# SimonsRoad/gf-pl-slam

Hardware: AMD Instinct MI355X
Metric: stereo frames/sec (2k ORB + 500 LBD, 10 GN iters) (higher is better)
Workload: dtype f64

## Files before the change

gf-pl-slam_amd/csrc/gfpl_abi.hip:

```cpp
#include <hip/hip_runtime.h>

#include <algorithm>
#include <atomic>
#include <cmath>
#include <mutex>
#include <cstdio>
#include <cstdlib>
#include <cstring>
#include <vector>

#include "../../include/gfpl.h"
#include "gfpl_kernels.hpp"

using namespace gfpl;

#define GFPL_NEV 10

struct gfpl_ctx {
    int device = 0;
    hipStream_t stream = nullptr;
    bool own_stream = false;
    gfpl_camera cam{};
    gfpl_config cfg{};
    bool has_cam = false, has_cfg = false;
    bool timing = false;
    hipEvent_t ev[GFPL_NEV]{};
    float stage_ms[7]{};
    std::vector<gfpl_seqbatch*> sbs;
    std::atomic<int> n_detectors{0};
    std::mutex host_mu;
};

struct gfpl_seqbatch {
    gfpl_ctx* ctx = nullptr;
    int B = 0, kp_cap = 0, kl_cap = 0, mpt_cap = 0, mls_cap = 0;
    void* base = nullptr;
    int64_t bytes = 0;
    DevFrame slot[2];
    int prev_slot = 0;
    bool initialized = false;
    bool has_curr = false;
    DevTrack tr{};
    DevScratch scr{};
    void* stage[2] = {nullptr, nullptr};
    size_t stage_bytes[2] = {0, 0};
    gfpl_frames stage_view[2]{};
    hipStream_t copy = nullptr;
    hipEvent_t ev_ready[2]{}, ev_free[2]{};
    bool ready_pending[2] = {false, false}, free_recorded[2] = {false, false};
    hipEvent_t ev_ticket[16]{};
    int64_t n_tickets = 0;
    int32_t* last_n_pt = nullptr;
    int32_t* last_n_ls = nullptr;
    PyrBuild* pyrb = nullptr;
    int last_cut_mode = -1;
};

struct gfpl_event {
    int device = 0;
    hipEvent_t ev = nullptr;
    int64_t records = 0;
};

int gfpl_ctx_device(const gfpl_ctx* c) { return c->device; }
void* gfpl_ctx_stream(const gfpl_ctx* c) { return (void*)c->stream; }
const gfpl_camera* gfpl_ctx_camera(const gfpl_ctx* c) { return c->has_cam ? &c->cam : nullptr; }
int64_t gfpl_event_records(const gfpl_event* e) { return e->records; }
void gfpl_ctx_attach(gfpl_ctx* c) { c->n_detectors.fetch_add(1); }
void gfpl_ctx_detach(gfpl_ctx* c) { c->n_detectors.fetch_sub(1); }


namespace {

#define HIPCHK(x)                                                  \
    do {                                                            \
        hipError_t e_ = (x);                                        \
        if (e_ != hipSuccess) {                                     \
            std::fprintf(stderr, "gfpl: %s failed: %s\n", #x, hipGetErrorString(e_)); \
            return GFPL_E_HIP;                                      \
        }                                                           \
    } while (0)

int debug_fill_byte() {
    const char* e = getenv("GFPL_DEBUG_FILL");
    return e ? (int)(strtol(e, nullptr, 0) & 0xFF) : 0;
}

template <typename F, typename H, typename V>
void frame_fields(F& f, H& o, V& v) {
    v.pt(f.pt.pl, o.pt_pl, 2); v.pt(f.pt.pl_obs, o.pt_pl_obs, 2);
    v.pt(f.pt.disp, o.pt_disp, 1); v.pt(f.pt.P, o.pt_P, 3); v.pt(f.pt.sigma2, o.pt_sigma2, 1);
    v.pt(f.pt.idx, o.pt_idx, 1); v.pt(f.pt.level, o.pt_level, 1); v.pt(f.pt.inlier, o.pt_inlier, 1);
    v.pt(f.pt.desc, o.pdesc, 32); v.count(f.pt.n);
    v.ls(f.ls.spl, o.ls_spl, 2); v.ls(f.ls.epl, o.ls_epl, 2);
    v.ls(f.ls.spl_obs, o.ls_spl_obs, 2); v.ls(f.ls.epl_obs, o.ls_epl_obs, 2);
    v.ls(f.ls.sdisp, o.ls_sdisp, 1); v.ls(f.ls.edisp, o.ls_edisp, 1);
    v.ls(f.ls.sdisp_obs, o.ls_sdisp_obs, 1); v.ls(f.ls.edisp_obs, o.ls_edisp_obs, 1);
    v.ls(f.ls.angle, o.ls_angle, 1); v.ls(f.ls.sigma2, o.ls_sigma2, 1);
    v.ls(f.ls.sP, o.ls_sP, 3); v.ls(f.ls.eP, o.ls_eP, 3);
    v.ls(f.ls.le, o.ls_le, 3); v.ls(f.ls.le_obs, o.ls_le_obs, 3);
    v.ls(f.ls.covS, o.ls_covS, 9); v.ls(f.ls.covE, o.ls_covE, 9);
    v.ls(f.ls.cut, o.ls_cut, 2); v.ls(f.ls.invcov, o.ls_invcov, 36);
    v.ls(f.ls.idx, o.ls_idx, 1); v.ls(f.ls.level, o.ls_level, 1); v.ls(f.ls.inlier, o.ls_inlier, 1);
    v.ls(f.ls.desc, o.ldesc, 32); v.count(f.ls.n);
    v.seq(f.pose.Tfw, o.Tfw, 16); v.seq(f.pose.DT, o.DT, 16);
    v.seq(f.pose.DT_cov, o.DT_cov, 36); v.seq(f.pose.Tfw_cov, o.Tfw_cov, 36);
    v.seq(f.pose.DT_cov_eig, o.DT_cov_eig, 6);
    v.seq(f.pose.err_norm, &o.err_norm, 1); v.seq(f.pose.time_stamp, &o.time_stamp, 1);
}

struct SlotCarve {
    Carver& c;
    size_t B, P, L;
    template <typename T, typename U> void pt(T*& d, U, int w) { d = c.take<T>(P * w); }
// ... 240 lines not shown

int gfpl_event_record(gfpl_event* e, gfpl_ctx* c) {
    if (!e || !c || e->device != c->device) return GFPL_E_INVALID;
    HIPCHK(hipEventRecord(e->ev, c->stream));
    ++e->records;
    return GFPL_OK;
}

int gfpl_event_wait(gfpl_ctx* c, gfpl_event* e) {
    if (!e || !c || e->device != c->device) return GFPL_E_INVALID;
    HIPCHK(hipStreamWaitEvent(c->stream, e->ev, 0));
    return GFPL_OK;
}

int gfpl_event_synchronize(gfpl_event* e) {
    if (!e) return GFPL_E_INVALID;
    HIPCHK(hipEventSynchronize(e->ev));
    return GFPL_OK;
}

int gfpl_set_camera(gfpl_ctx* c, const gfpl_camera* cam) {
    if (!c || !cam || cam->n_levels < 1 || cam->n_levels > GFPL_MAX_LEVELS) return GFPL_E_INVALID;
    if (!c->sbs.empty() || c->n_detectors.load() != 0) return GFPL_E_STATE;
    int64_t need = 0;
    for (int i = 0; i < cam->n_levels; ++i) {
        if (cam->lvl_cols[i] < 1 || cam->lvl_rows[i] < 1 || cam->lvl_offset[i] < 0) return GFPL_E_INVALID;
        if (cam->lvl_cols[i] > GFPL_MAX_IMAGE_DIM || cam->lvl_rows[i] > GFPL_MAX_IMAGE_DIM) return GFPL_E_INVALID;
        need = std::max<int64_t>(need, cam->lvl_offset[i] + (int64_t)cam->lvl_cols[i] * cam->lvl_rows[i]);
    }
    if (cam->pyr_bytes < need + GFPL_PYR_TAIL) return GFPL_E_INVALID;
    if (cam->pyr_bytes % 4 != 0) return GFPL_E_INVALID;
    c->cam = *cam;
    c->has_cam = true;
    return GFPL_OK;
}

int gfpl_set_config(gfpl_ctx* c, const gfpl_config* cfg) {
    if (!c || !cfg) return GFPL_E_INVALID;
    int e = cfg_supported(*cfg);
    if (e) return e;
    for (const gfpl_seqbatch* sb : c->sbs)
        if (cfg->max_point_match_num > sb->mpt_cap || cfg->max_line_match_num > sb->mls_cap) return GFPL_E_CAPACITY;
    c->cfg = *cfg;
    c->has_cfg = true;
    return GFPL_OK;
}

int gfpl_get_camera(const gfpl_ctx* c, gfpl_camera* cam) {
    if (!c || !cam || !c->has_cam) return GFPL_E_INVALID;
    *cam = c->cam;
    return GFPL_OK;
}

int gfpl_get_config(const gfpl_ctx* c, gfpl_config* cfg) {
    if (!c || !cfg) return GFPL_E_INVALID;
    *cfg = c->cfg;
    return GFPL_OK;
}

int gfpl_synchronize(gfpl_ctx* c) {
    if (!c) return GFPL_E_INVALID;
    HIPCHK(hipStreamSynchronize(c->stream));
    return GFPL_OK;
}

int gfpl_seqbatch_create(gfpl_ctx* c, int batch, int kp_cap, int kl_cap, gfpl_seqbatch** out) {
    if (!c || !out || batch < 1 || kp_cap < 2 || kl_cap < 2 || kp_cap > 8192 || kl_cap > 2048 || !c->has_cam)
        return GFPL_E_INVALID;
    HIPCHK(hipSetDevice(c->device));
    gfpl_seqbatch* sb = new gfpl_seqbatch();
    sb->ctx = c;
    sb->B = batch;
    sb->kp_cap = (kp_cap + 1) & ~1;
    sb->kl_cap = (kl_cap + 1) & ~1;
    sb->mpt_cap = c->cfg.max_point_match_num;
    sb->mls_cap = c->cfg.max_line_match_num;
    Carver dry;
// ... 13 lines not shown
}

int gfpl_seqbatch_destroy(gfpl_seqbatch* sb) {
    if (!sb) return GFPL_E_INVALID;
    (void)hipStreamSynchronize(sb->ctx->stream);
    auto& v = sb->ctx->sbs;
    v.erase(std::remove(v.begin(), v.end(), sb), v.end());
    if (sb->copy) (void)hipStreamSynchronize(sb->copy);
    if (sb->base) (void)hipFree(sb->base);
    for (int k = 0; k < 2; ++k) {
        if (sb->stage[k]) (void)hipFree(sb->stage[k]);
        if (sb->ev_ready[k]) (void)hipEventDestroy(sb->ev_ready[k]);
        if (sb->ev_free[k]) (void)hipEventDestroy(sb->ev_free[k]);
    }
    for (hipEvent_t e : sb->ev_ticket)
        if (e) (void)hipEventDestroy(e);
    if (sb->copy) (void)hipStreamDestroy(sb->copy);
    pyrbuild_destroy(sb->pyrb);
    delete sb;
    return GFPL_OK;
}

int64_t gfpl_seqbatch_bytes(const gfpl_seqbatch* sb) { return sb ? sb->bytes : 0; }

int gfpl_initialize(gfpl_seqbatch* sb, const gfpl_frames* in) {
    if (!sb) return GFPL_E_INVALID;
    int e = check_in(sb, in);
    if (e) return e;
    const int slot = in_acquire(sb, in);
    if (slot == -2) return GFPL_E_HIP;
    KParams p = params(sb, in);
    p.curr = sb->slot[sb->prev_slot];
    HIPCHK(launch_init(p, sb->ctx->stream));
    sb->initialized = true;
    sb->has_curr = false;
    return in_release(sb, in, slot);
}

int gfpl_stereo_points(gfpl_seqbatch* sb, const gfpl_frames* in) {
    if (!sb) return GFPL_E_INVALID;
    if (!sb->initialized) return GFPL_E_STATE;
    int e = check_in(sb, in);
    if (e) return e;
    const int slot = in_acquire(sb, in);
    if (slot == -2) return GFPL_E_HIP;
    HIPCHK(launch_stereo_points(params(sb, in), sb->ctx->stream));
    sb->has_curr = true;
    return in_release(sb, in, slot);
}

int gfpl_stereo_lines(gfpl_seqbatch* sb, const gfpl_frames* in) {
    if (!sb) return GFPL_E_INVALID;
    if (!sb->initialized) return GFPL_E_STATE;
    int e = check_in(sb, in);
    if (e) return e;
    const int slot = in_acquire(sb, in);
    if (slot == -2) return GFPL_E_HIP;
    HIPCHK(launch_stereo_lines(params(sb, in), sb->ctx->stream));
    sb->has_curr = true;
    return in_release(sb, in, slot);
}

int gfpl_line_uncertainty(gfpl_seqbatch* sb) {
    if (!sb) return GFPL_E_INVALID;
    if (!sb->initialized) return GFPL_E_STATE;
    HIPCHK(launch_line_uncertainty(params(sb, nullptr), sb->ctx->stream));
    return GFPL_OK;
}

int gfpl_cross_points(gfpl_seqbatch* sb) {
    if (!sb) return GFPL_E_INVALID;
    if (!sb->initialized || !sb->has_curr) return GFPL_E_STATE;
    HIPCHK(launch_cross_points(params(sb, nullptr), sb->ctx->stream));
    return GFPL_OK;
}

int gfpl_cross_lines(gfpl_seqbatch* sb) {
    if (!sb) return GFPL_E_INVALID;
    if (!sb->initialized || !sb->has_curr) return GFPL_E_STATE;
    HIPCHK(launch_cross_lines(params(sb, nullptr), sb->ctx->stream));
    return GFPL_OK;
}

int gfpl_line_cut(gfpl_seqbatch* sb) {
    if (!sb) return GFPL_E_INVALID;
    if (!sb->initialized || !sb->has_curr) return GFPL_E_STATE;
    sb->last_cut_mode = sb->ctx->cfg.cut_proof;
    HIPCHK(launch_line_cut(params(sb, nullptr), sb->ctx->stream, nullptr));
    return GFPL_OK;
}

int gfpl_insert_stereo_pair(gfpl_seqbatch* sb, const gfpl_frames* in) {
    if (!sb) return GFPL_E_INVALID;
    if (!sb->initialized) return GFPL_E_STATE;
    int e = check_in(sb, in);
    if (e) return e;
    gfpl_ctx* c = sb->ctx;
    const int slot = in_acquire(sb, in);
    if (slot == -2) return GFPL_E_HIP;
    KParams p = params(sb, in);
    tmark(c, 0);
    HIPCHK(launch_stereo_points(p, c->stream));
    tmark(c, 1);
    HIPCHK(launch_stereo_lines(p, c->stream));
    tmark(c, 2);
    if (c->cfg.use_line_conf_cut) HIPCHK(launch_line_uncertainty(p, c->stream));
    HIPCHK(launch_cross_points(p, c->stream));
    tmark(c, 3);
    HIPCHK(launch_cross_lines(p, c->stream));
    tmark(c, 4);
    sb->last_cut_mode = c->cfg.use_line_conf_cut ? c->cfg.cut_proof : -1;
    if (c->cfg.use_line_conf_cut)
        HIPCHK(launch_line_cut(p, c->stream, c->timing ? &c->ev[7] : nullptr));
    HIPCHK(launch_step_bytes(p, c->stream));
    tmark(c, 5);
    sb->has_curr = true;
    return in_release(sb, in, slot);
}

int gfpl_optimize_pose(gfpl_seqbatch* sb) {
    if (!sb) return GFPL_E_INVALID;
    if (!sb->initialized || !sb->has_curr) return GFPL_E_STATE;
    HIPCHK(launch_pose(params(sb, nullptr), sb->ctx->stream, sb->ctx->timing ? sb->ctx->ev[9] : nullptr));
    tmark(sb->ctx, 6);
    return GFPL_OK;
}

int gfpl_need_new_kf(gfpl_seqbatch* sb, int32_t* flags) {
    if (!sb) return GFPL_E_INVALID;
    if (!sb->initialized || !sb->has_curr) return GFPL_E_STATE;
    HIPCHK(launch_need_kf(params(sb, nullptr), sb->ctx->stream));
    if (flags) {
        HIPCHK(hipMemcpyAsync(flags, sb->tr.kf_flag, sizeof(int32_t) * (size_t)sb->B, hipMemcpyDeviceToHost,
                              sb->ctx->stream));
        HIPCHK(hipStreamSynchronize(sb->ctx->stream));
    }
    return GFPL_OK;
}

int gfpl_curr_frame_is_kf(gfpl_seqbatch* sb, const int32_t* mask) {
    if (!sb) return GFPL_E_INVALID;
    if (!sb->initialized || !sb->has_curr) return GFPL_E_STATE;
    const int32_t* dmask = sb->tr.kf_flag;
    if (mask) {
        HIPCHK(hipMemcpyAsync(sb->scr.kf_mask, mask, sizeof(int32_t) * (size_t)sb->B, hipMemcpyHostToDevice,
                              sb->ctx->stream));
// ... 498 lines not shown
    return GFPL_OK;
}
}

extern "C" {

int gfpl_read_frame(gfpl_seqbatch* sb, int which, int seq, gfpl_frame_host* o) {
    if (!sb || !o || seq < 0 || seq >= sb->B || (which != GFPL_PREV && which != GFPL_CURR)) return GFPL_E_INVALID;
    hipStream_t s = sb->ctx->stream;
    const DevFrame& f = sb->slot[which == GFPL_PREV ? sb->prev_slot : 1 - sb->prev_slot];
    HIPCHK(hipStreamSynchronize(s));
    int np = 0, nl = 0;
    HIPCHK(hipMemcpy(&np, f.pt.n + seq, 4, hipMemcpyDeviceToHost));
    HIPCHK(hipMemcpy(&nl, f.ls.n + seq, 4, hipMemcpyDeviceToHost));
    o->n_pt = np; o->n_ls = nl;
    SlotCopy<true> v{s, (size_t)seq, (size_t)seq * sb->kp_cap, (size_t)seq * sb->kl_cap, (size_t)np, (size_t)nl};
    frame_fields(f, *o, v);
    HIPCHK(v.e);
    HIPCHK(hipStreamSynchronize(s));
    return GFPL_OK;
}

int gfpl_write_frame(gfpl_seqbatch* sb, int which, int seq, const gfpl_frame_host* o) {
    if (!sb || !o || seq < 0 || seq >= sb->B || (which != GFPL_PREV && which != GFPL_CURR)) return GFPL_E_INVALID;
    if (o->n_pt < 0 || o->n_pt > sb->kp_cap || o->n_ls < 0 || o->n_ls > sb->kl_cap) return GFPL_E_CAPACITY;
    hipStream_t s = sb->ctx->stream;
    const DevFrame& f = sb->slot[which == GFPL_PREV ? sb->prev_slot : 1 - sb->prev_slot];
    XFER(h2d, f.pt.n + seq, &o->n_pt, 1);
    XFER(h2d, f.ls.n + seq, &o->n_ls, 1);
    SlotCopy<false> v{s, (size_t)seq, (size_t)seq * sb->kp_cap, (size_t)seq * sb->kl_cap, (size_t)o->n_pt, (size_t)o->n_ls};
    frame_fields(f, *o, v);
    HIPCHK(v.e);
    HIPCHK(hipStreamSynchronize(s));
    sb->initialized = true;
    if (which == GFPL_CURR) sb->has_curr = true;
    return GFPL_OK;
}

int gfpl_read_track(gfpl_seqbatch* sb, int seq, gfpl_track_host* o) {
    return read_track(sb, seq, o, sb ? sb->tr.n_matched_pt : nullptr, sb ? sb->tr.n_matched_ls : nullptr);
}

int gfpl_read_last_track(gfpl_seqbatch* sb, int seq, gfpl_track_host* o) {
    return read_track(sb, seq, o, sb ? sb->last_n_pt : nullptr, sb ? sb->last_n_ls : nullptr);
}

int gfpl_write_track(gfpl_seqbatch* sb, int seq, const gfpl_track_host* o) {
    if (!sb || !o || seq < 0 || seq >= sb->B) return GFPL_E_INVALID;
    if (o->n_matched_pt < 0 || o->n_matched_pt > sb->mpt_cap || o->n_matched_ls < 0 || o->n_matched_ls > sb->mls_cap)
        return GFPL_E_CAPACITY;
    hipStream_t s = sb->ctx->stream;
    XFER(h2d, sb->tr.n_matched_pt + seq, &o->n_matched_pt, 1);
    XFER(h2d, sb->tr.n_matched_ls + seq, &o->n_matched_ls, 1);
    XFER(h2d, sb->tr.n_inliers + seq, &o->n_inliers, 1);
    XFER(h2d, sb->tr.n_inliers_pt + seq, &o->n_inliers_pt, 1);
    XFER(h2d, sb->tr.n_inliers_ls + seq, &o->n_inliers_ls, 1);
    XFER(h2d, sb->tr.num_frame_loss + seq, &o->num_frame_loss, 1);
    XFER(h2d, sb->tr.matched_pt + (size_t)seq * sb->mpt_cap, o->matched_pt, (size_t)o->n_matched_pt);
    XFER(h2d, sb->tr.matched_ls + (size_t)seq * sb->mls_cap, o->matched_ls, (size_t)o->n_matched_ls);
    HIPCHK(hipStreamSynchronize(s));
    return GFPL_OK;
}

int gfpl_set_timing(gfpl_ctx* c, int enable) {
    if (!c) return GFPL_E_INVALID;
    c->timing = enable != 0;
// ... 59 lines not shown
    if (e) return e;
    for (int s = 0; s < 7; ++s) bytes7[s] = v[s];
    return GFPL_OK;
}

int gfpl_last_step_counts(gfpl_seqbatch* sb, int64_t* counts8) {
    if (!sb || !counts8) return GFPL_E_INVALID;
    int64_t v[STEP_REC];
    int e = step_rec_sums(sb, v);
    if (e) return e;
    for (int s = 0; s < 8; ++s) counts8[s] = v[8 + s];
    return GFPL_OK;
}

int gfpl_last_step_track_counts(gfpl_seqbatch* sb, int64_t* counts4) {
    if (!sb || !counts4) return GFPL_E_INVALID;
    int64_t v[STEP_REC];
    int e = step_rec_sums(sb, v);
    if (e) return e;
    for (int s = 0; s < 4; ++s) counts4[s] = v[16 + s];
    return GFPL_OK;
}

int gfpl_last_step_cut_proof(gfpl_seqbatch* sb, int64_t* counts4) {
    if (!sb || !counts4) return GFPL_E_INVALID;
    int64_t v[STEP_REC];
    int e = step_rec_sums(sb, v);
    if (e) return e;
    const bool on = sb->last_cut_mode == 1 || sb->last_cut_mode == 3;
    for (int s = 0; s < 4; ++s) counts4[s] = on ? v[20 + s] : 0;
    return GFPL_OK;
}

int gfpl_debug_cut_records(gfpl_seqbatch* sb, int b, double* out, int n_lines) {
    if (!sb || !out || b < 0 || b >= sb->B || n_lines < 0 || n_lines > sb->mls_cap) return GFPL_E_INVALID;
    if (hipSetDevice(sb->ctx->device) != hipSuccess) return GFPL_E_HIP;
    if (hipStreamSynchronize(sb->ctx->stream) != hipSuccess) return GFPL_E_HIP;
    const size_t n = (size_t)n_lines * CUT_REC;
    return hipMemcpy(out, sb->scr.cut_rec + (size_t)b * sb->mls_cap * CUT_REC, n * sizeof(double),
                     hipMemcpyDeviceToHost) == hipSuccess ? GFPL_OK : GFPL_E_HIP;
}

int gfpl_debug_step_records(gfpl_seqbatch* sb, int64_t* out) {
    if (!sb || !out) return GFPL_E_INVALID;
    if (hipSetDevice(sb->ctx->device) != hipSuccess) return GFPL_E_HIP;
    if (hipStreamSynchronize(sb->ctx->stream) != hipSuccess) return GFPL_E_HIP;
    return hipMemcpy(out, sb->scr.bytes, (size_t)sb->B * STEP_REC * sizeof(int64_t), hipMemcpyDeviceToHost) == hipSuccess
               ? GFPL_OK : GFPL_E_HIP;
}

int gfpl_debug_clocks(gfpl_seqbatch* sb, int64_t* out) {
    if (!sb || !out) return GFPL_E_INVALID;
    if (hipSetDevice(sb->ctx->device) != hipSuccess) return GFPL_E_HIP;
    if (hipStreamSynchronize(sb->ctx->stream) != hipSuccess) return GFPL_E_HIP;
    return hipMemcpy(out, sb->scr.dbg, (size_t)sb->B * 8 * sizeof(int64_t), hipMemcpyDeviceToHost) == hipSuccess
               ? GFPL_OK : GFPL_E_HIP;
}

int gfpl_last_step_bytes(gfpl_seqbatch* sb, int64_t* bytes) {
    if (!bytes) return GFPL_E_INVALID;
    int64_t v[7];
    int e = gfpl_last_step_stage_bytes(sb, v);
    if (e) return e;
    *bytes = v[6];
    return GFPL_OK;
}
// ... 3 lines not shown
```

gf-pl-slam_amd/csrc/k_stereo.hip:

```cpp
#include <type_traits>

#include "gfpl_kernels.hpp"
#include "gfpl_knn.hpp"

namespace gfpl {

template <typename K>
__device__ void bitonic_sort(K* a, int n) {
    for (int k = 2; k <= n; k <<= 1)
        for (int j = k >> 1; j > 0; j >>= 1) {
            for (int i = threadIdx.x; i < n; i += blockDim.x) {
                int ixj = i ^ j;
                if (ixj > i) {
                    bool up = ((i & k) == 0);
                    K x = a[i], y = a[ixj];
                    if ((x > y) == up) { a[i] = y; a[ixj] = x; }
                }
            }
            __syncthreads();
        }
}

template <typename K>
__device__ void bitonic_sort2(K* a, K* c, int n) {
// ... 105 lines not shown
        for (int s = 0; s < 11; ++s) {
            uint32_t a = acc[s];
#pragma unroll
            for (int k = 0; k < 5; ++k) a = __builtin_amdgcn_sad_u16(ILp[k] + cRR[s], RP[s + 2 * k], a);
            const uint32_t rt = (s + 10 < 19 ? RP[s + 10] : pair16(R, s + 10) + cLL) & 0xFFFFu;
            a = __builtin_amdgcn_sad_u16(il10 + (cRR[s] & 0xFFFFu), rt, a);
            acc[s] = a;
        }
    }
}

__device__ __forceinline__ void sad_finish(const KParams& p, const SadJob& J, float xL,
                                           const uint32_t* acc, float& disparity, float& bestuR) {
    int bestDist = 2147483647;
    int bestinc = 0;
    float vD[11];
#pragma unroll
    for (int s = 0; s < 11; ++s) {
        float dist = (float)(int)acc[s];
        if (dist < (float)bestDist) { bestDist = (int)dist; bestinc = s - 5; }
        vD[s] = dist;
    }
    if (bestinc == -5 || bestinc == 5) return;
    const float dist1 = vD[5 + bestinc - 1];
    const float dist2 = vD[5 + bestinc];
    const float dist3 = vD[5 + bestinc + 1];
    const float deltaR = (dist1 - dist3) / (2.0f * (dist1 + dist3 - 2.0f * dist2));
    if (deltaR < -1 || deltaR > 1) return;
    bestuR = p.cam.scale[J.o] * ((float)J.scaleduR0 + (float)bestinc + deltaR);
    disparity = (xL - bestuR);
}

#ifndef GFPL_SL_WAVES
#define GFPL_SL_WAVES 1
#endif
#ifndef GFPL_SP_WAVES
#define GFPL_SP_WAVES 6
#endif
#ifndef GFPL_SP_TY
#define GFPL_SP_TY 3
#endif
#ifndef GFPL_SP_TX
#define GFPL_SP_TX 6
#endif

__device__ __forceinline__ void wave_lds_sync() { asm volatile("s_waitcnt lgkmcnt(0)" ::: "memory"); }
#ifndef GFPL_SP_PRIO
#define GFPL_SP_PRIO 1
#endif
#if GFPL_SP_PRIO
#define SP_PRIO(k) __builtin_amdgcn_s_setprio(k)
#else
#define SP_PRIO(k) do { } while (0)
#endif
#ifdef GFPL_SP_CLOCK
#define SP_CLK(k) do { if (threadIdx.x == 0) p.scr.dbg[8 * (size_t)blockIdx.x + (k)] = (int64_t)wall_clock64(); } while (0)
#else
#define SP_CLK(k) do { } while (0)
#endif
template <int BLOCK, bool SEG>
__global__ void __launch_bounds__(BLOCK, GFPL_SP_WAVES) k_stereo_points(KParams p, int KP2) {
    extern __shared__ __align__(16) unsigned char smem[];
    const int b = blockIdx.x;
    const int cap = p.kp_cap;
    const int nRows = p.cam.height;
    const int nlev = p.cam.n_levels;
    const StereoPointsLds S(smem, KP2, nRows, nlev, SEG, BLOCK / 64);
// ... 537 lines not shown
    double epx = (-(le_r[2] + le_r[1] * (double)a.ey)) / le_r[0];
    double disp_s = (double)a.sx - spx;
    double disp_e = (double)a.ex - epx;
    double horiz = initial ? (double)fabsf((float)le_r[0]) : (double)fabsf((float)le_l[0]);
    if (!(disp_s >= p.cfg.min_disp && disp_e >= p.cfg.min_disp && horiz > p.cfg.line_horiz_th &&
          overlap > p.cfg.stereo_overlap_th))
        return false;
    if (!initial) {
        double cS[9], cE[9];
        endpointCov(cam, sp_l[0], sp_l[1], disp_s, cS);
        endpointCov(cam, ep_l[0], ep_l[1], disp_e, cE);
        const double th = p.cfg.line_cov_th;
        const int gS = eig_gate_bound(cS, th), gE = eig_gate_bound(cE, th);
        if (gS == 0 || gE == 0) return false;
        if (!(gS == 1 && gE == 1)) {
            double wS[3], wE[3];
            eig_sym<3>(cS, wS);
            eig_sym<3>(cE, wE);
            double max_eig = std_max(wS[2], wE[2]);
            if (!(max_eig < th)) return false;
        }
    }
    L->spl[0] = sp_l[0]; L->spl[1] = sp_l[1];
    L->epl[0] = ep_l[0]; L->epl[1] = ep_l[1];
    L->sdisp = disp_s; L->edisp = disp_e;
    backProjection(cam, sp_l[0], sp_l[1], disp_s, L->sP);
    backProjection(cam, ep_l[0], ep_l[1], disp_e, L->eP);
    L->le[0] = le_l[0]; L->le[1] = le_l[1]; L->le[2] = le_l[2];
    L->angle = (double)a.angle;
    L->level = a.octave;
    return true;
}

__device__ void line_uncertainty(const KParams& p, const double* spl, const double* epl, double sdisp,
                                 double edisp, const double* le, double* covS, double* covE) {
    double sdisp_std, edisp_std;
    if (fabs(le[0]) > 0.15) {
        sdisp_std = p.cfg.ratio_disp_std * sdisp;
        edisp_std = p.cfg.ratio_disp_std * edisp;
    } else {
        sdisp_std = p.cfg.ratio_disp_std_hor * sdisp;
        edisp_std = p.cfg.ratio_disp_std_hor * edisp;
    }
    covMat2D_3D(p.cam, spl[0], spl[1], 1.0, sdisp, sdisp_std, covS);
    covMat2D_3D(p.cam, epl[0], epl[1], 1.0, edisp, edisp_std, covE);
}

__device__ void write_line(const KParams& p, DevLines& C, size_t q, const LineOut& L, int idx, const uint8_t* desc) {
    C.spl[2 * q] = L.spl[0]; C.spl[2 * q + 1] = L.spl[1];
    C.epl[2 * q] = L.epl[0]; C.epl[2 * q + 1] = L.epl[1];
    C.sdisp[q] = L.sdisp; C.edisp[q] = L.edisp;
    for (int k = 0; k < 3; ++k) { C.sP[3 * q + k] = L.sP[k]; C.eP[3 * q + k] = L.eP[k]; C.le[3 * q + k] = L.le[k]; }
    C.angle[q] = L.angle;
    C.level[q] = L.level;
    C.sigma2[q] = p.cam.sigma2_ln[clamp_level(L.level, GFPL_MAX_LEVELS)];
    C.idx[q] = idx;
    C.inlier[q] = 1;
    C.cut[2 * q] = 0.0; C.cut[2 * q + 1] = 0.0;
    const uint4* s = reinterpret_cast<const uint4*>(desc);
    uint4* d = reinterpret_cast<uint4*>(C.desc + q * 32);
    d[0] = s[0]; d[1] = s[1];
}

template <int CELL>
__device__ __forceinline__ void knn2_row(const uint32_t* q, const uint32_t* T, int nt, int& i0, int& d0, int& d1) {
    int dist0 = 2147483647, dist1 = 2147483647, idx0 = -1;
    for (int j = 0; j < nt; ++j) {
        const int d = hamming8<CELL>(q, T + 8 * j);
        if (d < dist1) {
            if (dist0 > d) { dist1 = dist0; dist0 = d; idx0 = j; }
            else { dist1 = d; }
        }
    }
    i0 = idx0; d0 = dist0; d1 = dist1;
}

#ifdef GFPL_SL_CLOCK
#define SL_CLK(k) do { if (threadIdx.x == 0 && !INITIAL) p.scr.dbg[8 * (size_t)blockIdx.x + (k)] = (int64_t)wall_clock64(); } while (0)
#else
#define SL_CLK(k) do { } while (0)
#endif
template <int CELL, bool INITIAL, int BLOCK>
__global__ void __launch_bounds__(BLOCK, GFPL_SL_WAVES) k_stereo_lines(KParams p) {
    extern __shared__ __align__(16) unsigned char smem[];
    const int b = blockIdx.x;
    const int cap = p.kl_cap;
    uint32_t* lut = (uint32_t*)smem;
    uint32_t* tb = lut + knn_lut_dwords(CELL);
    int* lr_i = (int*)(tb + cap * 8);
    int* lr_d0 = lr_i + cap;
    int* lr_d1 = lr_d0 + cap;
    int* rl_i = lr_d1 + cap;
    int* hist = rl_i + cap;
    int* misc = hist + 260;
    const int tid = threadIdx.x;
    const int NL = min(p.in.n_kl_l[b], cap), NR = min(p.in.n_kl_r[b], cap);
    DevLines& C = p.curr.ls;
    if (NL < 2 || NR < 2) {
        if (tid == 0) C.n[b] = 0;
        return;
    }
    const uint8_t* DLg = p.in.ldesc_l + (size_t)b * cap * 32;
    const uint8_t* DRg = p.in.ldesc_r + (size_t)b * cap * 32;
    SL_CLK(0);
    SL_PRIO(3);
    knn_stage_views<CELL>(tb, cap, DRg, NR);
    for (int i = tid; i < 260; i += blockDim.x) hist[i] = 0;
    for (int j = tid; j < NR; j += blockDim.x) rl_i[j] = -1;
    knn_lut_fill<CELL>(lut);
    __syncthreads();
    SL_CLK(1);
    knn2_mfma<CELL, true, true, true>(tb, cap, NR, DLg, NL, (uint32_t*)lr_i, (uint32_t*)lr_d1, lut, (uint32_t*)rl_i);
    __syncthreads();
    SL_CLK(2);
    SL_PRIO(1);
    for (int i = tid; i < NL; i += blockDim.x) {
// ... 2 lines not shown
        lr_i[i] = (int)(k0 & 0xFFFFu); lr_d0[i] = d0; lr_d1[i] = d1;
        atomicAdd(&hist[d1 - d0], 1);
    }
    for (int j = tid; j < NR; j += blockDim.x) rl_i[j] = (int)((uint32_t)rl_i[j] & 0xFFFFu);
    __syncthreads();
    if (tid < 64) {
        const int v = wave_hist_rank(hist, NL / 2, 257);
        if (tid == 0) {
            double th = (1.4826 * (double)(float)v) * p.cfg.desc_th_l;
            reinterpret_cast<double*>(misc + 8)[0] = th;
        }
    }
    __syncthreads();
    const double nn12_dist_th = reinterpret_cast<double*>(misc + 8)[0];
    SL_CLK(3);
    const int n_matches = min(NL, NR);
    const gfpl_keyline* KL = p.in.kl_l + (size_t)b * cap;
    const gfpl_keyline* KR = p.in.kl_r + (size_t)b * cap;
    const size_t base = (size_t)b * cap;
    int off = 0;
    for (int c0 = 0; c0 < n_matches; c0 += BLOCK) {
        const int i = c0 + tid;
        int flag = 0;
        LineOut L;
        if (i < n_matches) {
            const int lr_tdx = lr_i[i];
            const int rl_tdx = rl_i[lr_tdx];
            const double dist_12 = (double)((float)lr_d1[i] - (float)lr_d0[i]);
            if (i == rl_tdx && dist_12 > nn12_dist_th)
                flag = triangulate(p, KL[i], KR[lr_tdx], INITIAL, &L) ? 1 : 0;
        }
        int tot;
        const int pos = off + block_exclusive_scan<BLOCK>(flag, misc + 16, &tot);
        if (flag) write_line(p, C, base + pos, L, INITIAL ? pos : -1, DLg + (size_t)i * 32);
        off += tot;
    }
    if (tid == 0) C.n[b] = off;
    SL_CLK(4);
}

template <int CELL>
__global__ void __launch_bounds__(256) k_knn2(const uint8_t* q, const int* nq_arr, int nq_fixed, size_t q_stride,
                                             const uint8_t* t, const int* nt_arr, int nt_fixed, size_t t_stride,
                                             int cap_clamp, int32_t* out_idx, float* out_dist, int32_t* packed,
                                             size_t out_stride) {
    const int b = blockIdx.y;
    const int nq = nq_arr ? min(nq_arr[b], cap_clamp) : nq_fixed;
    const int nt = nt_arr ? min(nt_arr[b], cap_clamp) : nt_fixed;
    const int i = blockIdx.x * blockDim.x + threadIdx.x;
    if (i >= nq) return;
    const uint8_t* Q = q + (size_t)b * q_stride * 32;
    const uint8_t* T = t + (size_t)b * t_stride * 32;
    uint32_t qd[8];
    load_desc(Q + (size_t)i * 32, qd);
    int dist0 = 2147483647, dist1 = 2147483647, idx0 = -1, idx1 = -1;
    for (int j = 0; j < nt; ++j) {
        uint32_t td[8];
        load_desc(T + (size_t)j * 32, td);
        const int d = hamming8<CELL>(qd, td);
        if (d < dist1) {
            if (dist0 > d) { dist1 = dist0; idx1 = idx0; dist0 = d; idx0 = j; }
            else { dist1 = d; idx1 = j; }
        }
    }
    if (out_idx) {
        out_idx[2 * i] = idx0; out_idx[2 * i + 1] = idx1;
        out_dist[2 * i] = (float)dist0; out_dist[2 * i + 1] = (float)dist1;
// ... 247 lines not shown
```

gf-pl-slam_amd/gfpl/__init__.py:

```python
from __future__ import annotations

import ctypes as C
import json
import os
from typing import Optional

import numpy as np

PKG_DIR = os.path.dirname(os.path.dirname(os.path.abspath(__file__)))
LIB_DIR = os.path.join(PKG_DIR, "lib")
REPO_DIR = os.path.dirname(PKG_DIR)

DESC = 32
MAX_LEVELS = 8
MAX_MATCHED_PT = 2048
MAX_MATCHED_LS = 1024
PREV, CURR = 0, 1
HAMMING, HAMMING2 = 1, 2

ERRORS = {0: "ok", -1: "invalid argument", -2: "HIP runtime error", -3: "no HIP device",
          -4: "knn-2 needs at least 2 train descriptors", -5: "capacity exceeded",
          -6: "call order violated", -7: "unsupported config", -8: "device memory allocation failed"}


# ... 279 lines not shown
            "gfpl_update_frame": ([P], C.c_int),
            "gfpl_frame_step": ([P, P], C.c_int),
            "gfpl_upload_frames": ([P, P, P], C.c_int),
            "gfpl_upload_frames_async": ([P, P, C.c_int, C.c_int, P], C.c_int),
            "gfpl_upload_wait": ([P, C.c_int64], C.c_int),
            "gfpl_upload_frames_l0_async": ([P, P, C.c_int, C.c_int, C.c_int64, P], C.c_int),
            "gfpl_staged_frames": ([P, C.c_int, P], C.c_int),
            "gfpl_stereo_points": ([P, P], C.c_int),
            "gfpl_stereo_lines": ([P, P], C.c_int),
            "gfpl_line_uncertainty": ([P], C.c_int),
            "gfpl_cross_points": ([P], C.c_int),
            "gfpl_cross_lines": ([P], C.c_int),
            "gfpl_line_cut": ([P], C.c_int),
            "gfpl_knn2_hamming": ([P, P, C.c_int, P, C.c_int, C.c_int, P, P], C.c_int),
            "gfpl_kf_common_matches": ([P, P, P, P, P, P, P], C.c_int),
            "gfpl_kf_local_map_matches": ([P, P, P, C.c_double, C.c_double, P, P, P, P], C.c_int),
            "gfpl_read_frame": ([P, C.c_int, C.c_int, P], C.c_int),
            "gfpl_write_frame": ([P, C.c_int, C.c_int, P], C.c_int),
            "gfpl_read_track": ([P, C.c_int, P], C.c_int),
            "gfpl_read_last_track": ([P, C.c_int, P], C.c_int),
            "gfpl_need_new_kf": ([P, P], C.c_int),
            "gfpl_curr_frame_is_kf": ([P, P], C.c_int),
            "gfpl_read_kf_state": ([P, C.c_int, P], C.c_int),
            "gfpl_write_track": ([P, C.c_int, P], C.c_int),
            "gfpl_set_timing": ([P, C.c_int], C.c_int),
            "gfpl_get_stage_times": ([P, P], C.c_int),
            "gfpl_get_kernel_times": ([P, P], C.c_int),
            "gfpl_last_step_kernel_bytes": ([P, P], C.c_int),
            "gfpl_last_step_bytes": ([P, P], C.c_int),
            "gfpl_last_step_stage_bytes": ([P, P], C.c_int),
            "gfpl_last_step_counts": ([P, P], C.c_int),
            "gfpl_last_step_track_counts": ([P, P], C.c_int),
            "gfpl_last_step_cut_proof": ([P, P], C.c_int),
            "gfpl_debug_cut_records": ([P, C.c_int, P, C.c_int], C.c_int),
            "gfpl_debug_step_records": ([P, P], C.c_int),
            "gfpl_debug_clocks": ([P, P], C.c_int),
            "gfpl_lsd_create": ([P, P, C.c_int, C.c_int, C.c_int, C.c_int, C.c_int, C.POINTER(P)], C.c_int),
            "gfpl_lsd_destroy": ([P], C.c_int),
            "gfpl_lsd_detect": ([P, P, C.c_int, P, P, P], C.c_int),
            "gfpl_lsd_sort_desc": ([P, P, C.c_int], C.c_int),
            "gfpl_strerror": ([C.c_int], C.c_char_p),
            "gfpl_orb_create": ([P, C.c_int, C.c_int, P, C.c_int, C.c_int, C.POINTER(P)], C.c_int),
            "gfpl_orb_destroy": ([P], C.c_int),
            "gfpl_orb_pyramid_bytes": ([P, P], C.c_int),
            "gfpl_orb_extract": ([P, P, C.c_int, P, P, P, P, P, P, C.c_int64], C.c_int),
            "gfpl_lbd_create": ([P, C.c_int, C.c_int, C.c_int, C.c_int, C.POINTER(P)], C.c_int),
            "gfpl_lbd_destroy": ([P], C.c_int),
            "gfpl_lbd_compute": ([P, P, C.c_int, P, P, P], C.c_int),
            "gfpl_lbd_gradients": ([P, P, P], C.c_int),
            "gfpl_detector_params_default": ([P, P, P], C.c_int),
            "gfpl_detector_create": ([P, P, C.c_int, C.c_int, C.c_int, C.c_int, C.POINTER(P)], C.c_int),
            "gfpl_detector_destroy": ([P], C.c_int),
            "gfpl_detect_stereo_async": ([P, P, P, C.c_int, P, P], C.c_int),
            "gfpl_detect_stereo_host": ([P, P, P, C.c_int, P, P], C.c_int),
            "gfpl_detect_stereo": ([P, P, P, C.c_int, P, C.c_int, P], C.c_int),
            "gfpl_detector_status": ([P], C.c_int),
            "gfpl_detector_discard": ([P, P], C.c_int),
            "gfpl_read_detections": ([P, P, C.c_int, P], C.c_int),
            "gfpl_rectify_maps_host": ([P, C.c_int, C.c_int, P, P], C.c_int),
            "gfpl_rectifier_create": ([P, P, P, C.c_int, C.c_int, C.POINTER(P)], C.c_int),
            "gfpl_rectifier_destroy": ([P], C.c_int),
            "gfpl_rectifier_read_maps": ([P, C.c_int, P, P], C.c_int),
            "gfpl_rectify": ([P, C.c_int, P, C.c_int, P], C.c_int),
            "gfpl_rectify_async": ([P, C.c_int, P, C.c_int, P], C.c_int),
            "gfpl_rectify_stereo_async": ([P, P, P, C.c_int, P, P], C.c_int),
            "gfpl_rectify_host": ([P, C.c_int, P, C.c_int, P], C.c_int),
# ... 540 lines not shown
        return st.as_dict()

    def write_track(self, seq: int, tr: TrackHost):
        check(self.L.gfpl_write_track(self.h, seq, C.byref(tr)), "write_track")

    def last_step_bytes(self) -> int:
        v = C.c_int64()
        check(self.L.gfpl_last_step_bytes(self.h, C.byref(v)), "last_step_bytes")
        return v.value

    def last_step_stage_bytes(self) -> np.ndarray:
        v = np.zeros(7, np.int64)
        check(self.L.gfpl_last_step_stage_bytes(self.h, v.ctypes.data), "last_step_stage_bytes")
        return v

    STEP_COUNTS = ["N_o", "N_k", "M_o", "S_p", "S_l", "M_p", "M_l", "n_inliers"]

    def last_step_counts(self) -> dict:
        v = np.zeros(8, np.int64)
        check(self.L.gfpl_last_step_counts(self.h, v.ctypes.data), "last_step_counts")
        return {n: float(x) / self.B for n, x in zip(self.STEP_COUNTS, v)}

    def last_step_track_counts(self) -> dict:
        v = np.zeros(4, np.int64)
        check(self.L.gfpl_last_step_track_counts(self.h, v.ctypes.data), "last_step_track_counts")
        return {"steps": int(v[0]), "exact_steps": int(v[1]), "inliers_after_pose": int(v[2]),
                "lines_unbounded": int(v[3])}

    def last_step_cut_proof(self) -> dict:
        v = np.zeros(4, np.int64)
        check(self.L.gfpl_last_step_cut_proof(self.h, v.ctypes.data), "last_step_cut_proof")
        return {"redone": int(v[0]), "steps_proven": int(v[1]), "vref_evals": int(v[2]), "lines": int(v[3])}

    def debug_cut_records(self, b: int, n_lines: int) -> np.ndarray:
        out = np.zeros((n_lines, 80), np.float64)
        check(self.L.gfpl_debug_cut_records(self.h, b, out.ctypes.data, n_lines), "debug_cut_records")
        return out

    def debug_step_records(self) -> np.ndarray:
        out = np.zeros((self.B, 24), np.int64)
        check(self.L.gfpl_debug_step_records(self.h, out.ctypes.data), "debug_step_records")
        return out

    def debug_clocks(self) -> np.ndarray:
        out = np.zeros((self.B, 8), np.int64)
        check(self.L.gfpl_debug_clocks(self.h, out.ctypes.data), "debug_clocks")
        return out

    def last_step_kernel_bytes(self) -> np.ndarray:
        v = np.zeros(4, np.int64)
        check(self.L.gfpl_last_step_kernel_bytes(self.h, v.ctypes.data), "last_step_kernel_bytes")
        return v

    def nbytes(self) -> int:
        return int(self.L.gfpl_seqbatch_bytes(self.h))

    def close(self):
        if getattr(self, "h", None):
            self.L.gfpl_seqbatch_destroy(self.h)
            self.h = None

    def __del__(self):
        try:
            self.close()
        except Exception:
            pass
# ... 373 lines not shown
```

include/gfpl.h:

```cpp
#ifndef GFPL_H
#define GFPL_H

#include <stddef.h>
#include <stdint.h>

#ifdef __cplusplus
extern "C" {
#endif

#define GFPL_ABI_VERSION 6

#define GFPL_DESC_BYTES 32
#define GFPL_MAX_LEVELS 8
#define GFPL_MAX_IMAGE_DIM 2047
#define GFPL_MAX_MATCHED_PT 2048
#define GFPL_MAX_MATCHED_LS 1024
#define GFPL_PYR_TAIL 64

#define GFPL_OK                   0
#define GFPL_E_INVALID          (-1)
#define GFPL_E_HIP              (-2)
#define GFPL_E_NO_DEVICE        (-3)
#define GFPL_E_TOO_FEW_TRAIN    (-4)
#define GFPL_E_CAPACITY         (-5)
// ... 318 lines not shown
    const double*  ls_sigma2;
    double         T_kf_w[16];
} gfpl_kf_view;

int  gfpl_kf_common_matches(gfpl_ctx* ctx, const gfpl_kf_view* kf0, const gfpl_kf_view* kf1,
                            int32_t* pt_pairs, int* n_pt_pairs, int32_t* ls_pairs, int* n_ls_pairs);

typedef struct gfpl_map_view {
    int            n_pt;
    const uint8_t* pdesc;
    const double*  P;
    int            n_ls;
    const uint8_t* ldesc;
    const double*  L;
} gfpl_map_view;

int  gfpl_kf_local_map_matches(gfpl_ctx* ctx, const gfpl_map_view* map, const gfpl_kf_view* kf1,
                               double max_kf_epip_p, double max_kf_epip_l,
                               int32_t* pt_pairs, int* n_pt_pairs, int32_t* ls_pairs, int* n_ls_pairs);

int  gfpl_read_frame(gfpl_seqbatch* sb, int which, int seq, gfpl_frame_host* out);
int  gfpl_write_frame(gfpl_seqbatch* sb, int which, int seq, const gfpl_frame_host* in);
int  gfpl_read_track(gfpl_seqbatch* sb, int seq, gfpl_track_host* out);
int  gfpl_write_track(gfpl_seqbatch* sb, int seq, const gfpl_track_host* in);
int  gfpl_read_last_track(gfpl_seqbatch* sb, int seq, gfpl_track_host* out);

int  gfpl_set_timing(gfpl_ctx* ctx, int enable);
int  gfpl_get_stage_times(gfpl_ctx* ctx, float* ms7);
int  gfpl_last_step_bytes(gfpl_seqbatch* sb, int64_t* bytes);
int  gfpl_last_step_stage_bytes(gfpl_seqbatch* sb, int64_t* bytes7);
int  gfpl_last_step_counts(gfpl_seqbatch* sb, int64_t* counts8);
int  gfpl_last_step_track_counts(gfpl_seqbatch* sb, int64_t* counts4);
int  gfpl_last_step_cut_proof(gfpl_seqbatch* sb, int64_t* counts4);
int  gfpl_debug_cut_records(gfpl_seqbatch* sb, int b, double* out, int n_lines);
int  gfpl_debug_step_records(gfpl_seqbatch* sb, int64_t* out);
int  gfpl_debug_clocks(gfpl_seqbatch* sb, int64_t* out);
int  gfpl_get_kernel_times(gfpl_ctx* ctx, float* ms4);
int  gfpl_last_step_kernel_bytes(gfpl_seqbatch* sb, int64_t* bytes4);

const char* gfpl_strerror(int code);

#ifdef __cplusplus
}
#endif
#endif
```

Baseline: 781,100.

## Fuse line covariance into stereo-lines kernel and skip redundant uncertainty launches

The stereo-lines kernel now writes each line's start and end 3D covariances as it writes the line, when the confidence cut is enabled. A per-slot generation mark records that the covariances are current, so the step skips the separate line-uncertainty launch on the previous frame when they were already produced. Launch-bound occupancy hints for the stereo-lines kernel also change per block size and mode. This saves a kernel launch and a reread of line data, but adds register pressure and extra bookkeeping that must be invalidated correctly whenever config, camera, or frame writes change.

```diff
diff --git a/gf-pl-slam_amd/csrc/gfpl_abi.hip b/gf-pl-slam_amd/csrc/gfpl_abi.hip
--- a/gf-pl-slam_amd/csrc/gfpl_abi.hip
+++ b/gf-pl-slam_amd/csrc/gfpl_abi.hip
@@ -24,6 +24,7 @@
     gfpl_config cfg{};
     bool has_cam = false, has_cfg = false;
     bool timing = false;
+    int64_t cov_gen = 0;
     hipEvent_t ev[GFPL_NEV]{};
     float stage_ms[7]{};
     std::vector<gfpl_seqbatch*> sbs;
@@ -38,6 +39,8 @@
     int64_t bytes = 0;
     DevFrame slot[2];
     int prev_slot = 0;
+    int64_t cov_mark[2] = {-1, -1};
+    int64_t n_line_unc = 0;
     bool initialized = false;
     bool has_curr = false;
     DevTrack tr{};
@@ -80,6 +83,11 @@
             return GFPL_E_HIP;                                      \
         }                                                           \
     } while (0)
+
+void mark_lines_written(gfpl_seqbatch* sb, int slot) {
+    sb->cov_mark[slot] = sb->ctx->cfg.use_line_conf_cut ? sb->ctx->cov_gen : -1;
+}
+bool cov_current(const gfpl_seqbatch* sb, int slot) { return sb->cov_mark[slot] == sb->ctx->cov_gen; }
 
 int debug_fill_byte() {
     const char* e = getenv("GFPL_DEBUG_FILL");
@@ -386,6 +394,7 @@
     if (cam->pyr_bytes % 4 != 0) return GFPL_E_INVALID;
     c->cam = *cam;
     c->has_cam = true;
+    ++c->cov_gen;
     return GFPL_OK;
 }
 
@@ -397,6 +406,7 @@
         if (cfg->max_point_match_num > sb->mpt_cap || cfg->max_line_match_num > sb->mls_cap) return GFPL_E_CAPACITY;
     c->cfg = *cfg;
     c->has_cfg = true;
+    ++c->cov_gen;
     return GFPL_OK;
 }
 
@@ -476,6 +486,7 @@
     KParams p = params(sb, in);
     p.curr = sb->slot[sb->prev_slot];
     HIPCHK(launch_init(p, sb->ctx->stream));
+    mark_lines_written(sb, sb->prev_slot);
     sb->initialized = true;
     sb->has_curr = false;
     return in_release(sb, in, slot);
@@ -500,7 +511,10 @@
     if (e) return e;
     const int slot = in_acquire(sb, in);
     if (slot == -2) return GFPL_E_HIP;
-    HIPCHK(launch_stereo_lines(params(sb, in), sb->ctx->stream));
+    KParams p = params(sb, in);
+    p.cfg.use_line_conf_cut = 0;
+    HIPCHK(launch_stereo_lines(p, sb->ctx->stream));
+    sb->cov_mark[1 - sb->prev_slot] = -1;
     sb->has_curr = true;
     return in_release(sb, in, slot);
 }
@@ -509,6 +523,8 @@
     if (!sb) return GFPL_E_INVALID;
     if (!sb->initialized) return GFPL_E_STATE;
     HIPCHK(launch_line_uncertainty(params(sb, nullptr), sb->ctx->stream));
+    ++sb->n_line_unc;
+    sb->cov_mark[sb->prev_slot] = sb->ctx->cov_gen;
     return GFPL_OK;
 }
 
@@ -531,6 +547,7 @@
     if (!sb->initialized || !sb->has_curr) return GFPL_E_STATE;
     sb->last_cut_mode = sb->ctx->cfg.cut_proof;
     HIPCHK(launch_line_cut(params(sb, nullptr), sb->ctx->stream, nullptr));
+    sb->cov_mark[sb->prev_slot] = -1;
     return GFPL_OK;
 }
 
@@ -547,15 +564,22 @@
     HIPCHK(launch_stereo_points(p, c->stream));
     tmark(c, 1);
     HIPCHK(launch_stereo_lines(p, c->stream));
+    mark_lines_written(sb, 1 - sb->prev_slot);
     tmark(c, 2);
-    if (c->cfg.use_line_conf_cut) HIPCHK(launch_line_uncertainty(p, c->stream));
+    if (c->cfg.use_line_conf_cut && !cov_current(sb, sb->prev_slot)) {
+        HIPCHK(launch_line_uncertainty(p, c->stream));
+        ++sb->n_line_unc;
+        sb->cov_mark[sb->prev_slot] = c->cov_gen;
+    }
     HIPCHK(launch_cross_points(p, c->stream));
     tmark(c, 3);
     HIPCHK(launch_cross_lines(p, c->stream));
     tmark(c, 4);
     sb->last_cut_mode = c->cfg.use_line_conf_cut ? c->cfg.cut_proof : -1;
-    if (c->cfg.use_line_conf_cut)
+    if (c->cfg.use_line_conf_cut) {
         HIPCHK(launch_line_cut(p, c->stream, c->timing ? &c->ev[7] : nullptr));
+        sb->cov_mark[sb->prev_slot] = -1;
+    }
     HIPCHK(launch_step_bytes(p, c->stream));
     tmark(c, 5);
     sb->has_curr = true;
@@ -1120,6 +1144,7 @@
     frame_fields(f, *o, v);
     HIPCHK(v.e);
     HIPCHK(hipStreamSynchronize(s));
+    sb->cov_mark[which == GFPL_PREV ? sb->prev_slot : 1 - sb->prev_slot] = -1;
     sb->initialized = true;
     if (which == GFPL_CURR) sb->has_curr = true;
     return GFPL_OK;
@@ -1245,6 +1270,19 @@
     return GFPL_OK;
 }
 
+int64_t gfpl_debug_line_uncertainty_launches(const gfpl_seqbatch* sb) { return sb ? sb->n_line_unc : -1; }
+
+int gfpl_debug_line_cov_rows(gfpl_seqbatch* sb, int which, int seq, double* covS, double* covE) {
+    if (!sb || !covS || !covE || seq < 0 || seq >= sb->B || (which != GFPL_PREV && which != GFPL_CURR)) return GFPL_E_INVALID;
+    if (hipSetDevice(sb->ctx->device) != hipSuccess) return GFPL_E_HIP;
+    if (hipStreamSynchronize(sb->ctx->stream) != hipSuccess) return GFPL_E_HIP;
+    const DevLines& L = sb->slot[which == GFPL_PREV ? sb->prev_slot : 1 - sb->prev_slot].ls;
+    const size_t n = 9 * (size_t)sb->kl_cap, off = n * (size_t)seq;
+    HIPCHK(hipMemcpy(covS, L.covS + off, n * sizeof(double), hipMemcpyDeviceToHost));
+    HIPCHK(hipMemcpy(covE, L.covE + off, n * sizeof(double), hipMemcpyDeviceToHost));
+    return GFPL_OK;
+}
+
 int gfpl_debug_cut_records(gfpl_seqbatch* sb, int b, double* out, int n_lines) {
     if (!sb || !out || b < 0 || b >= sb->B || n_lines < 0 || n_lines > sb->mls_cap) return GFPL_E_INVALID;
     if (hipSetDevice(sb->ctx->device) != hipSuccess) return GFPL_E_HIP;
diff --git a/gf-pl-slam_amd/csrc/k_stereo.hip b/gf-pl-slam_amd/csrc/k_stereo.hip
--- a/gf-pl-slam_amd/csrc/k_stereo.hip
+++ b/gf-pl-slam_amd/csrc/k_stereo.hip
@@ -161,7 +161,7 @@
 }
 
 #ifndef GFPL_SL_WAVES
-#define GFPL_SL_WAVES 1
+#define GFPL_SL_WAVES(BLOCK, INITIAL) ((INITIAL) ? 5 : ((BLOCK) == 512 ? 4 : 1))
 #endif
 #ifndef GFPL_SP_WAVES
 #define GFPL_SP_WAVES 6
@@ -765,16 +765,20 @@
     return true;
 }
 
-__device__ void line_uncertainty(const KParams& p, const double* spl, const double* epl, double sdisp,
-                                 double edisp, const double* le, double* covS, double* covE) {
-    double sdisp_std, edisp_std;
-    if (fabs(le[0]) > 0.15) {
+__device__ __forceinline__ void line_disp_std(const KParams& p, double le0, double sdisp, double edisp,
+                                              double& sdisp_std, double& edisp_std) {
+    if (fabs(le0) > 0.15) {
         sdisp_std = p.cfg.ratio_disp_std * sdisp;
         edisp_std = p.cfg.ratio_disp_std * edisp;
     } else {
         sdisp_std = p.cfg.ratio_disp_std_hor * sdisp;
         edisp_std = p.cfg.ratio_disp_std_hor * edisp;
     }
+}
+__device__ void line_uncertainty(const KParams& p, const double* spl, const double* epl, double sdisp,
+                                 double edisp, const double* le, double* covS, double* covE) {
+    double sdisp_std, edisp_std;
+    line_disp_std(p, le[0], sdisp, edisp, sdisp_std, edisp_std);
     covMat2D_3D(p.cam, spl[0], spl[1], 1.0, sdisp, sdisp_std, covS);
     covMat2D_3D(p.cam, epl[0], epl[1], 1.0, edisp, edisp_std, covE);
 }
@@ -795,6 +799,19 @@
     d[0] = s[0]; d[1] = s[1];
 }
 
+__device__ __forceinline__ void write_line_cov(const KParams& p, DevLines& C, size_t q, const LineOut& L) {
+    double sdisp_std, edisp_std, c[9];
+    line_disp_std(p, L.le[0], L.sdisp, L.edisp, sdisp_std, edisp_std);
+    asm volatile("" ::: "memory");
+    covMat2D_3D(p.cam, L.spl[0], L.spl[1], 1.0, L.sdisp, sdisp_std, c);
+#pragma unroll
+    for (int k = 0; k < 9; ++k) C.covS[9 * q + k] = c[k];
+    asm volatile("" ::: "memory");
+    covMat2D_3D(p.cam, L.epl[0], L.epl[1], 1.0, L.edisp, edisp_std, c);
+#pragma unroll
+    for (int k = 0; k < 9; ++k) C.covE[9 * q + k] = c[k];
+}
+
 template <int CELL>
 __device__ __forceinline__ void knn2_row(const uint32_t* q, const uint32_t* T, int nt, int& i0, int& d0, int& d1) {
     int dist0 = 2147483647, dist1 = 2147483647, idx0 = -1;
@@ -814,7 +831,7 @@
 #define SL_CLK(k) do { } while (0)
 #endif
 template <int CELL, bool INITIAL, int BLOCK>
-__global__ void __launch_bounds__(BLOCK, GFPL_SL_WAVES) k_stereo_lines(KParams p) {
+__global__ void __launch_bounds__(BLOCK, GFPL_SL_WAVES(BLOCK, INITIAL)) k_stereo_lines(KParams p) {
     extern __shared__ __align__(16) unsigned char smem[];
     const int b = blockIdx.x;
     const int cap = p.kl_cap;
@@ -883,7 +900,10 @@
         }
         int tot;
         const int pos = off + block_exclusive_scan<BLOCK>(flag, misc + 16, &tot);
-        if (flag) write_line(p, C, base + pos, L, INITIAL ? pos : -1, DLg + (size_t)i * 32);
+        if (flag) {
+            write_line(p, C, base + pos, L, INITIAL ? pos : -1, DLg + (size_t)i * 32);
+            if (p.cfg.use_line_conf_cut) write_line_cov(p, C, base + pos, L);
+        }
         off += tot;
     }
     if (tid == 0) C.n[b] = off;
diff --git a/gf-pl-slam_amd/gfpl/__init__.py b/gf-pl-slam_amd/gfpl/__init__.py
--- a/gf-pl-slam_amd/gfpl/__init__.py
+++ b/gf-pl-slam_amd/gfpl/__init__.py
@@ -335,6 +335,8 @@
             "gfpl_last_step_counts": ([P, P], C.c_int),
             "gfpl_last_step_track_counts": ([P, P], C.c_int),
             "gfpl_last_step_cut_proof": ([P, P], C.c_int),
+            "gfpl_debug_line_uncertainty_launches": ([P], C.c_int64),
+            "gfpl_debug_line_cov_rows": ([P, C.c_int, C.c_int, P, P], C.c_int),
             "gfpl_debug_cut_records": ([P, C.c_int, P, C.c_int], C.c_int),
             "gfpl_debug_step_records": ([P, P], C.c_int),
             "gfpl_debug_clocks": ([P, P], C.c_int),
@@ -941,6 +943,14 @@
         check(self.L.gfpl_last_step_cut_proof(self.h, v.ctypes.data), "last_step_cut_proof")
         return {"redone": int(v[0]), "steps_proven": int(v[1]), "vref_evals": int(v[2]), "lines": int(v[3])}
 
+    def line_uncertainty_launches(self) -> int:
+        return int(self.L.gfpl_debug_line_uncertainty_launches(self.h))
+
+    def debug_line_cov_rows(self, which: int, seq: int):
+        cs, ce = np.zeros((self.kl_cap, 9), np.float64), np.zeros((self.kl_cap, 9), np.float64)
+        check(self.L.gfpl_debug_line_cov_rows(self.h, which, seq, cs.ctypes.data, ce.ctypes.data), "debug_line_cov_rows")
+        return cs, ce
+
     def debug_cut_records(self, b: int, n_lines: int) -> np.ndarray:
         out = np.zeros((n_lines, 80), np.float64)
         check(self.L.gfpl_debug_cut_records(self.h, b, out.ctypes.data, n_lines), "debug_cut_records")
diff --git a/include/gfpl.h b/include/gfpl.h
--- a/include/gfpl.h
+++ b/include/gfpl.h
@@ -374,6 +374,8 @@
 int  gfpl_last_step_counts(gfpl_seqbatch* sb, int64_t* counts8);
 int  gfpl_last_step_track_counts(gfpl_seqbatch* sb, int64_t* counts4);
 int  gfpl_last_step_cut_proof(gfpl_seqbatch* sb, int64_t* counts4);
+int64_t gfpl_debug_line_uncertainty_launches(const gfpl_seqbatch* sb);
+int  gfpl_debug_line_cov_rows(gfpl_seqbatch* sb, int which, int seq, double* covS, double* covE);
 int  gfpl_debug_cut_records(gfpl_seqbatch* sb, int b, double* out, int n_lines);
 int  gfpl_debug_step_records(gfpl_seqbatch* sb, int64_t* out);
 int  gfpl_debug_clocks(gfpl_seqbatch* sb, int64_t* out);
```

Measured after the change: 786,900 (median of 6 runs). No clear change (+0.7%).
